# etzinis/sudo_rm_rf

Hardware: NVIDIA H100
Metric: mixtures_per_sec_forward_4s_8kHz_2src (higher is better)
Workload: dtype f32

## Files before the change

### sudo_rm_rf_b200/csrc/pointwise_mma.cu

```cuda
#include <cstdio>
#include <cstdlib>
#include <cstring>
#include <mutex>
#include <vector>
#include <cuda.h>
#include <cuda_bf16.h>
#include "common.cuh"

namespace sdr {

constexpr int kTileM = 128;
constexpr int kTileN = 128;
constexpr int kBlockK = 64;
constexpr int kStages = 3;
constexpr int kRawStages = 2;
constexpr int kBoxL = 32;
constexpr int kBoxBytes = 64 * kBoxL * 4;
constexpr int kRawStageBytes = kTileM / kBoxL * kBoxBytes;
constexpr int kBHalf = kTileN * 128;
constexpr int kBStageBytes = 2 * kBHalf;
constexpr int kSlotBytes = 2 * kBoxBytes;
constexpr int kSlots = 4;
constexpr int kConsWarps = 8, kTmaWarp = 8, kRawWarp = 9, kGatherWarps = 2;
template <bool WINDOW> constexpr int kMmaThreads = 32 * (kRawWarp + (WINDOW ? kGatherWarps : 1));

struct MmaArgs {
    const float* x;
    NormIn nin;
    const float* bias;
    int gate_channels;
    float* y;
    double* stats_out;
    int M, K, L;
    int l_tiles, n_tiles;
    int num_tiles;
    int epilogue;
    int win_k;
    int win_hop, win_pad, win_a;
    long long win_T;
};

__device__ __forceinline__ uint32_t smem_u32(const void* p) {
    return static_cast<uint32_t>(__cvta_generic_to_shared(p));
}
__device__ __forceinline__ void mbar_init(uint64_t* bar, uint32_t count) {
    asm volatile("mbarrier.init.shared::cta.b64 [%0], %1;" ::"r"(smem_u32(bar)), "r"(count) : "memory");
}
// ... 18 lines not shown
    asm volatile("fence.mbarrier_init.release.cluster;" ::: "memory");
}
__device__ __forceinline__ void fence_proxy_async_smem() {
    asm volatile("fence.proxy.async.shared::cta;" ::: "memory");
}
__device__ __forceinline__ void tma_load_2d(void* smem_dst, const CUtensorMap* tm, uint64_t* bar, int c0, int c1) {
    asm volatile("cp.async.bulk.tensor.2d.shared::cluster.global.tile.mbarrier::complete_tx::bytes [%0], [%1, {%3, %4}], [%2];"
                 ::"r"(smem_u32(smem_dst)), "l"(tm), "r"(smem_u32(bar)), "r"(c0), "r"(c1) : "memory");
}
__device__ __forceinline__ void tma_load_3d(void* smem_dst, const CUtensorMap* tm, uint64_t* bar, int c0, int c1, int c2) {
    asm volatile("cp.async.bulk.tensor.3d.shared::cluster.global.tile.mbarrier::complete_tx::bytes [%0], [%1, {%3, %4, %5}], [%2];"
                 ::"r"(smem_u32(smem_dst)), "l"(tm), "r"(smem_u32(bar)), "r"(c0), "r"(c1), "r"(c2) : "memory");
}
__device__ __forceinline__ void tma_store_3d(const CUtensorMap* tm, const void* smem_src, int c0, int c1, int c2) {
    asm volatile("cp.async.bulk.tensor.3d.global.shared::cta.bulk_group [%0, {%2, %3, %4}], [%1];"
                 ::"l"(tm), "r"(smem_u32(smem_src)), "r"(c0), "r"(c1), "r"(c2) : "memory");
}
__device__ __forceinline__ void bulk_commit() { asm volatile("cp.async.bulk.commit_group;" ::: "memory"); }
__device__ __forceinline__ void bulk_wait_read_all() { asm volatile("cp.async.bulk.wait_group.read 0;" ::: "memory"); }
__device__ __forceinline__ void bulk_wait_all() { asm volatile("cp.async.bulk.wait_group 0;" ::: "memory"); }
__device__ __forceinline__ void named_bar_sync(uint32_t id, uint32_t threads) {
    asm volatile("bar.sync %0, %1;" ::"r"(id), "r"(threads) : "memory");
}

__device__ __forceinline__ uint64_t gmma_desc_sw128(uint32_t saddr, uint32_t lbo, uint32_t sbo) {
    uint64_t d = 0;
    d |= (uint64_t)((saddr >> 4) & 0x3FFF);
    d |= (uint64_t)((lbo >> 4) & 0x3FFF) << 16;
    d |= (uint64_t)((sbo >> 4) & 0x3FFF) << 32;
    d |= (uint64_t)1 << 62;
    return d;
}
constexpr uint32_t kBLbo = 16, kBSbo = 1024;

__device__ __forceinline__ void wgmma_fence() { asm volatile("wgmma.fence.sync.aligned;" ::: "memory"); }
__device__ __forceinline__ void wgmma_commit() { asm volatile("wgmma.commit_group.sync.aligned;" ::: "memory"); }
template <int N>
__device__ __forceinline__ void wgmma_wait() { asm volatile("wgmma.wait_group.sync.aligned %0;" ::"n"(N) : "memory"); }
__device__ __forceinline__ void wgmma_bf16_m64n128_rs(float (&d)[64], const uint32_t (&a)[4], uint64_t bdesc,
                                                      uint32_t accumulate) {
    asm volatile(
        "{\n\t.reg .pred p;\n\t"
        "setp.ne.b32 p, %69, 0;\n\t"
        "wgmma.mma_async.sync.aligned.m64n128k16.f32.bf16.bf16 "
        "{%0, %1, %2, %3, %4, %5, %6, %7, %8, %9, %10, %11, %12, %13, %14, %15, %16, %17, %18, %19, %20, %21, %22, "
        "%23, %24, %25, %26, %27, %28, %29, %30, %31, %32, %33, %34, %35, %36, %37, %38, %39, %40, %41, %42, %43, %44, "
// ... 27 lines not shown
#pragma unroll
    for (int e = 0; e < 8; ++e) {
        const int k = kc * 8 + e;
        const float v = (m < M && k < Kreal) ? W[(size_t)m * Kreal + k] : 0.f;
        hi[e] = __float2bfloat16_rn(v);
        lo[e] = __float2bfloat16_rn(v - __bfloat162float(hi[e]));
    }
    *reinterpret_cast<uint4*>(img + off) = *reinterpret_cast<const uint4*>(hi);
    *reinterpret_cast<uint4*>(img + kBHalf + off) = *reinterpret_cast<const uint4*>(lo);
}

struct TileCoord { int sample, l0, n0; };
__device__ __forceinline__ TileCoord decode_tile(const MmaArgs& a, int tile) {
    TileCoord t;
    const int pos = tile / a.n_tiles;
    t.n0 = (tile - pos * a.n_tiles) * kTileN;
    t.sample = pos / a.l_tiles;
    t.l0 = (pos - t.sample * a.l_tiles) * kTileM;
    return t;
}

constexpr int kGroupSteps = 2;
constexpr int kGroups = kBlockK / 16 / kGroupSteps;
static_assert(kGroups == 2, "group g of every k-block uses fragment buffer g");
struct AFrag { uint32_t hi[kGroupSteps][4], lo[kGroupSteps][4]; };

template <bool WINDOW, int ACT, int MODE, bool STATS>
__global__ void __launch_bounds__(kMmaThreads<WINDOW>, 1)
pw_mma_kernel(const MmaArgs a, const __grid_constant__ CUtensorMap wmap,
              const __grid_constant__ CUtensorMap xmap,
              const __grid_constant__ CUtensorMap emap,
              const __grid_constant__ CUtensorMap ymap) {
    static_assert(!(WINDOW && ACT != 0), "the encoder's window operand has no activation");
    extern __shared__ uint8_t smem_raw[];
    uint8_t* smem = smem_raw + ((1024u - (smem_u32(smem_raw) & 1023u)) & 1023u);
    uint8_t* r_base = smem;
    uint8_t* b_base = r_base + kRawStages * kRawStageBytes;
    uint8_t* slots = b_base + kStages * kBStageBytes;
    float2* s_ab = reinterpret_cast<float2*>(slots + kSlots * kSlotBytes);
    float* s_sl = reinterpret_cast<float*>(s_ab + kRawStages * kBlockK);
    uint64_t* bars = reinterpret_cast<uint64_t*>(s_sl + kRawStages * kBlockK);
    uint64_t* full_bar = bars;
    uint64_t* empty_bar = full_bar + kStages;
    uint64_t* rfull_bar = empty_bar + kStages;
    uint64_t* rempty_bar = rfull_bar + kRawStages;
    uint64_t* slot_bar = rempty_bar + kRawStages;

    const int tid = threadIdx.x;
    const int warp = tid >> 5, lane = tid & 31;
    const int KB = a.K / kBlockK;
    const int tile0 = (int)blockIdx.x;
    const int tstep = (int)gridDim.x;

    if (warp == kTmaWarp && lane == 0) {
        for (int s = 0; s < kStages; ++s) { mbar_init(&full_bar[s], 1); mbar_init(&empty_bar[s], kConsWarps); }
        for (int s = 0; s < kRawStages; ++s) {
            mbar_init(&rfull_bar[s], WINDOW ? kGatherWarps : 2);
            mbar_init(&rempty_bar[s], kConsWarps);
        }
        for (int s = 0; s < kSlots; ++s) mbar_init(&slot_bar[s], 1);
        fence_barrier_init();
    }
    __syncthreads();

    if (warp >= kRawWarp) {
        int rs = 0;
        uint32_t rphase = 0;
        if constexpr (WINDOW) {
            constexpr int kGatherCh = kBlockK / kGatherWarps;
            const int c0 = (warp - kRawWarp) * kGatherCh;
#pragma unroll 1
            for (int tile = tile0; tile < a.num_tiles; tile += tstep) {
                const TileCoord tc = decode_tile(a, tile);
#pragma unroll 1
                for (int kb = 0; kb < KB; ++kb) {
                    uint8_t* rp = r_base + (size_t)rs * kRawStageBytes + (lane & 3) * 4;
#pragma unroll
                    for (int i0 = 0; i0 < kGatherCh; i0 += 16) {
                        float v[16][kTileM / kBoxL];
#pragma unroll
                        for (int i = 0; i < 16; ++i) {
                            const int k = kb * kBlockK + c0 + i0 + i;
                            const int ch = k / a.win_k, j = k - ch * a.win_k;
                            const float* src = a.x + ((size_t)tc.sample * a.win_a + ch) * a.win_T;
#pragma unroll
                            for (int b = 0; b < kTileM / kBoxL; ++b) {
                                const int l = tc.l0 + b * kBoxL + lane;
                                const long long t = (long long)a.win_hop * l + j - a.win_pad;
                                v[i][b] = (l < a.L && ch < a.win_a && t >= 0 && t < a.win_T) ? __ldg(src + t) : 0.f;
                            }
                        }
                        if (i0 == 0) mbar_wait(&rempty_bar[rs], rphase ^ 1);
#pragma unroll
                        for (int i = 0; i < 16; ++i) {
                            const int c = c0 + i0 + i;
#pragma unroll
                            for (int b = 0; b < kTileM / kBoxL; ++b)
                                *reinterpret_cast<float*>(rp + b * kBoxBytes + c * 128 + (((lane >> 2) ^ (c & 7)) << 4)) = v[i][b];
                        }
                    }
                    __syncwarp();
                    if (lane == 0) mbar_arrive(&rfull_bar[rs]);
                    if (++rs == kRawStages) { rs = 0; rphase ^= 1; }
                }
            }
        } else {
            const bool has_norm = a.nin.stats != nullptr;
            const double inv_count = 1.0 / a.nin.count;
#pragma unroll 1
            for (int tile = tile0; tile < a.num_tiles; tile += tstep) {
                const TileCoord tc = decode_tile(a, tile);
                float mean = 0.f, rstd = 1.f;
                if (has_norm) {
                    const double mu = a.nin.stats[2 * (size_t)tc.sample] * inv_count;
                    double var = a.nin.stats[2 * (size_t)tc.sample + 1] * inv_count - mu * mu;
                    var = var < 0.0 ? 0.0 : var;
                    mean = (float)mu;
                    rstd = rsqrtf((float)var + kGlnEps);
                }
#pragma unroll 1
                for (int kb = 0; kb < KB; ++kb) {
                    const int k = kb * kBlockK + 2 * lane;
                    float g[2] = {1.f, 1.f}, be[2] = {0.f, 0.f}, sl[2] = {1.f, 1.f};
                    if (has_norm) {
                        g[0] = __ldg(a.nin.gamma + k); g[1] = __ldg(a.nin.gamma + k + 1);
                        be[0] = __ldg(a.nin.beta + k); be[1] = __ldg(a.nin.beta + k + 1);
                    }
                    if constexpr (ACT == 2) { sl[0] = __ldg(a.nin.prelu + k); sl[1] = __ldg(a.nin.prelu + k + 1); }
                    mbar_wait(&rempty_bar[rs], rphase ^ 1);
                    if (lane == 0) {
                        mbar_arrive_expect_tx(&rfull_bar[rs], kRawStageBytes);
                        for (int b = 0; b < kTileM / kBoxL; ++b)
                            tma_load_3d(r_base + (size_t)rs * kRawStageBytes + b * kBoxBytes, &xmap, &rfull_bar[rs],
                                        tc.l0 + b * kBoxL, kb * kBlockK, tc.sample);
                    }
                    float aa[2] = {1.f, 1.f}, bb[2] = {0.f, 0.f};
                    if (has_norm) {
#pragma unroll
                        for (int e = 0; e < 2; ++e) { aa[e] = g[e] * rstd; bb[e] = be[e] - mean * aa[e]; }
                    }
                    *reinterpret_cast<float4*>(s_ab + rs * kBlockK + 2 * lane) = make_float4(aa[0], bb[0], aa[1], bb[1]);
                    if constexpr (ACT == 2) *reinterpret_cast<float2*>(s_sl + rs * kBlockK + 2 * lane) = make_float2(sl[0], sl[1]);
                    __syncwarp();
                    if (lane == 0) mbar_arrive(&rfull_bar[rs]);
                    if (++rs == kRawStages) { rs = 0; rphase ^= 1; }
                }
            }
        }
    } else if (warp == kTmaWarp) {
        if (lane == 0) {
            int stage = 0;
            uint32_t phase = 0;
            for (int tile = tile0; tile < a.num_tiles; tile += tstep) {
                const int nt = tile % a.n_tiles;
                for (int kb = 0; kb < KB; ++kb) {
                    mbar_wait(&empty_bar[stage], phase ^ 1);
                    mbar_arrive_expect_tx(&full_bar[stage], kBStageBytes);
                    tma_load_2d(b_base + (size_t)stage * kBStageBytes, &wmap, &full_bar[stage], 0, (nt * KB + kb) * 2 * kTileN);
                    if (++stage == kStages) { stage = 0; phase ^= 1; }
                }
            }
        }
        __syncwarp();
    } else {
        const int wg = warp >> 2;
        const int wr = warp & 3;
        const int q = lane & 3;
        const bool issuer = (tid & 127) == 0;
        const bool relu_out = WINDOW && a.epilogue == 2;
        const float slope = ACT == 1 ? __ldg(a.nin.prelu) : 1.f;
        const bool slope_le1 = slope <= 1.f;
        uint32_t boff[4];
#pragma unroll
        for (int v = 0; v < 4; ++v) {
            const uint32_t c = 2 * q + (v & 1), pp = 16 * (wr & 1) + (lane >> 2) + 8 * (v >> 1);
            boff[v] = c * 128 + (((pp >> 2) ^ c) << 4) + (pp & 3) * 4;
        }
        const uint32_t raw_box = (uint32_t)(2 * wg + (wr >> 1)) * kBoxBytes;
        uint8_t* const my_slots = slots + (size_t)(2 * wg) * kSlotBytes;
        auto fill_slot = [&](int tile, int h) {
            uint64_t* bar = &slot_bar[2 * wg + h];
            if constexpr (MODE == 0) {
                mbar_arrive(bar);
            } else {
                const TileCoord t = decode_tile(a, tile);
                const int c0 = t.l0 + 64 * wg;
                const int c1 = (MODE == 1 ? t.n0 : t.n0 % a.gate_channels) + 64 * h;
                uint8_t* const dst = my_slots + (size_t)h * kSlotBytes;
                mbar_arrive_expect_tx(bar, kSlotBytes);
                tma_load_3d(dst, &emap, bar, c0, c1, t.sample);
                tma_load_3d(dst + kBoxBytes, &emap, bar, c0 + kBoxL, c1, t.sample);
            }
        };
        if (issuer) { fill_slot(tile0, 0); fill_slot(tile0, 1); }

        int rs = 0, stage = 0, prev_stage = 0;
        uint32_t rphase = 0, phase = 0, slot_phase = 0;
        auto transform = [&](AFrag& f, int g) {
            if (g == 0) mbar_wait(&rfull_bar[rs], rphase);
            const uint8_t* rp = r_base + (size_t)rs * kRawStageBytes + raw_box;
            const float2* tab = s_ab + rs * kBlockK + 2 * q;
            const float* tsl = s_sl + rs * kBlockK + 2 * q;
#pragma unroll
            for (int s = 0; s < kGroupSteps; ++s) {
#pragma unroll
                for (int h = 0; h < 2; ++h) {
                    const int c = 16 * (g * kGroupSteps + s) + 8 * h;
                    float4 ab = make_float4(1.f, 0.f, 1.f, 0.f);
                    float2 sl = make_float2(1.f, 1.f);
                    if constexpr (!WINDOW) ab = *reinterpret_cast<const float4*>(tab + c);
                    if constexpr (ACT == 2) sl = *reinterpret_cast<const float2*>(tsl + c);
#pragma unroll
                    for (int ph = 0; ph < 2; ++ph) {
                        float y[2];
#pragma unroll
                        for (int e = 0; e < 2; ++e) {
                            const float x = *reinterpret_cast<const float*>(rp + boff[e + 2 * ph] + c * 128);
                            y[e] = WINDOW ? x : fmaf(x, e ? ab.z : ab.x, e ? ab.w : ab.y);
                            if constexpr (ACT == 1) {
                                const float t = y[e] * slope;
                                y[e] = slope_le1 ? fmaxf(y[e], t) : fminf(y[e], t);
                            } else if constexpr (ACT == 2) {
                                y[e] = y[e] >= 0.f ? y[e] : y[e] * (e ? sl.y : sl.x);
                            }
                        }
                        const uint32_t h0 = __float_as_uint(y[0]) & 0xffff0000u, h1 = __float_as_uint(y[1]) & 0xffff0000u;
                        const __nv_bfloat162 lo = __floats2bfloat162_rn(y[0] - __uint_as_float(h0), y[1] - __uint_as_float(h1));
                        f.hi[s][2 * h + ph] = __byte_perm(h0, h1, 0x7632);
                        f.lo[s][2 * h + ph] = *reinterpret_cast<const uint32_t*>(&lo);
                    }
                }
            }
            if (g == kGroups - 1) {
                __syncwarp();
                if (lane == 0) mbar_arrive(&rempty_bar[rs]);
                if (++rs == kRawStages) { rs = 0; rphase ^= 1; }
            }
        };
        float acc[64];
        auto mma_group = [&](int kb, int g, const AFrag& cur, AFrag& nxt) {
            if (g == 0) mbar_wait(&full_bar[stage], phase);
            const uint32_t sb_hi = smem_u32(b_base + (size_t)stage * kBStageBytes);
            const uint32_t sb_lo = sb_hi + kBHalf;
            wgmma_fence();
#pragma unroll
            for (int s = 0; s < kGroupSteps; ++s) {
                const int ks = g * kGroupSteps + s;
                const uint64_t dbh = gmma_desc_sw128(sb_hi + ks * 32, kBLbo, kBSbo);
                const uint64_t dbl = gmma_desc_sw128(sb_lo + ks * 32, kBLbo, kBSbo);
                wgmma_bf16_m64n128_rs(acc, cur.hi[s], dbh, (kb | ks) != 0 ? 1u : 0u);
                wgmma_bf16_m64n128_rs(acc, cur.lo[s], dbh, 1u);
                wgmma_bf16_m64n128_rs(acc, cur.hi[s], dbl, 1u);
            }
            wgmma_commit();
            wgmma_wait<1>();
            if (g == 0 && kb > 0) {
                __syncwarp();
                if (lane == 0) mbar_arrive(&empty_bar[prev_stage]);
            }
            if (g == kGroups - 1) {
                prev_stage = stage;
                if (++stage == kStages) { stage = 0; phase ^= 1; }
                if (kb + 1 < KB) transform(nxt, 0);
            } else {
                transform(nxt, g + 1);
            }
        };
        AFrag fa, fb;
#pragma unroll 1
        for (int tile = tile0; tile < a.num_tiles; tile += tstep) {
            const TileCoord tc = decode_tile(a, tile);
#pragma unroll
            for (int i = 0; i < 64; ++i) acc[i] = 0.f;
            transform(fa, 0);
#pragma unroll 1
            for (int kb = 0; kb < KB; ++kb) {
                mma_group(kb, 0, fa, fb);
                mma_group(kb, 1, fb, fa);
            }
            wgmma_wait<0>();
            __syncwarp();
            if (lane == 0) mbar_arrive(&empty_bar[prev_stage]);
            const int prem = a.L - (tc.l0 + wg * 64 + 32 * (wr >> 1) + 16 * (wr & 1) + (lane >> 2));
            StatAcc st;
            float rs_ = 0.f, rq = 0.f;
#pragma unroll
            for (int h = 0; h < 2; ++h) {
                uint8_t* const slot = my_slots + (size_t)h * kSlotBytes;
                uint8_t* const box = slot + (wr >> 1) * kBoxBytes;
                const int m0 = tc.n0 + 64 * h + 2 * q;
                const int mrem = a.M - m0;
                mbar_wait(&slot_bar[2 * wg + h], slot_phase);
#pragma unroll
                for (int j = 0; j < 8; ++j) {
                    float bv[2];
#pragma unroll
                    for (int b = 0; b < 2; ++b) bv[b] = (a.bias && 8 * j + b < mrem) ? __ldg(a.bias + m0 + 8 * j + b) : 0.f;
#pragma unroll
                    for (int v = 0; v < 4; ++v) {
                        const int u = 4 * j + v, i = 32 * h + u;
                        float* e = reinterpret_cast<float*>(box + boff[v] + 1024 * j);
                        float o = acc[i] + bv[v & 1];
                        if (MODE == 1) o += *e;
                        if (MODE == 2) o = fmaxf(o, 0.f) * *e;
                        if constexpr (WINDOW) { if (relu_out) o = fmaxf(o, 0.f); }
                        *e = o;
                        if (STATS && 8 * j + (v & 1) < mrem && 8 * (v >> 1) < prem) { rs_ += o; rq = fmaf(o, o, rq); }
                        if (STATS && (i & 15) == 15) { st.add_run(rs_, rq); rs_ = rq = 0.f; }
                    }
                }
                if constexpr (WINDOW) {
                    named_bar_sync(1 + wg, 128);
#pragma unroll 4
                    for (int r = wr; r < 64; r += 4) {
                        const int m = tc.n0 + 64 * h + r;
#pragma unroll
                        for (int half = 0; half < 2; ++half) {
                            const int p = tc.l0 + wg * 64 + half * kBoxL + lane;
                            const float v = *reinterpret_cast<const float*>(
                                slot + half * kBoxBytes + r * 128 + (((lane >> 2) ^ (r & 7)) << 4) + (lane & 3) * 4);
                            if (m < a.M && p < a.L) a.y[((size_t)tc.sample * a.M + m) * a.L + p] = v;
                        }
                    }
                    named_bar_sync(1 + wg, 128);
                } else {
                    fence_proxy_async_smem();
                    named_bar_sync(1 + wg, 128);
                    if (issuer) {
                        const int c0 = tc.l0 + wg * 64, c1 = tc.n0 + 64 * h;
                        tma_store_3d(&ymap, slot, c0, c1, tc.sample);
                        tma_store_3d(&ymap, slot + kBoxBytes, c0 + kBoxL, c1, tc.sample);
                        bulk_commit();
                        bulk_wait_read_all();
                    }
                }
                if (issuer && tile + tstep < a.num_tiles) fill_slot(tile + tstep, h);
            }
            slot_phase ^= 1;
            if (STATS) {
                const double ds = warp_sum_f64(st.s), dq = warp_sum_f64(st.q);
                if (lane == 0) {
                    atomicAdd(a.stats_out + 2 * (size_t)tc.sample, ds);
                    atomicAdd(a.stats_out + 2 * (size_t)tc.sample + 1, dq);
                }
            }
        }
        if (!WINDOW && issuer) bulk_wait_all();
    }
}

static inline int mma_pad_m(int M) { return (M + kTileN - 1) / kTileN * kTileN; }

bool pointwise_mma_eligible(int M, int K) {
    return M >= 32 && K >= kBlockK && (K % kBlockK) == 0;
}

size_t pointwise_mma_packed_bytes(int M, int K) {
    if (!pointwise_mma_eligible(M, K)) return 0;
    return (size_t)mma_pad_m(M) * K * 4;
}

// ... 39 lines not shown
                           CU_TENSOR_MAP_L2_PROMOTION_L2_256B, CU_TENSOR_MAP_FLOAT_OOB_FILL_NONE);
    return r == CUDA_SUCCESS ? SDR_OK : SDR_ERR_UNSUPPORTED;
}

static int make_act_map(CUtensorMap* tm, const float* x, int samples, int C, int L) {
    memset(tm, 0, sizeof(*tm));
    EncodeTiledFn enc = encode_tiled_fn();
    if (!enc) return SDR_ERR_CUDA;
    const cuuint64_t dims[3] = {(cuuint64_t)L, (cuuint64_t)C, (cuuint64_t)samples};
    const cuuint64_t strides[2] = {(cuuint64_t)L * 4, (cuuint64_t)L * C * 4};
    const cuuint32_t box[3] = {(cuuint32_t)kBoxL, 64, 1};
    const cuuint32_t estr[3] = {1, 1, 1};
    const CUresult r = enc(tm, CU_TENSOR_MAP_DATA_TYPE_FLOAT32, 3, const_cast<float*>(x), dims, strides, box, estr,
                           CU_TENSOR_MAP_INTERLEAVE_NONE, CU_TENSOR_MAP_SWIZZLE_128B,
                           CU_TENSOR_MAP_L2_PROMOTION_L2_256B, CU_TENSOR_MAP_FLOAT_OOB_FILL_NONE);
    return r == CUDA_SUCCESS ? SDR_OK : SDR_ERR_UNSUPPORTED;
}
static_assert(kBlockK == 64 && kTileN == 2 * 64, "activation boxes are 64 channels: one k-block, half a channel tile");

struct MmaLaunchInfo { const void* fn; int dev; int sms; };
static std::mutex g_launch_mutex;
static std::vector<MmaLaunchInfo> g_launch_info;

template <bool WINDOW, typename Kern>
static int launch_persistent(Kern kern, const MmaArgs& a, const CUtensorMap& wmap, const CUtensorMap& xmap,
                             const CUtensorMap& emap, const CUtensorMap& ymap, cudaStream_t st) {
    int dev = 0;
    if (cudaGetDevice(&dev) != cudaSuccess) return SDR_ERR_CUDA;
    int sms = 0;
    {
        std::lock_guard<std::mutex> lock(g_launch_mutex);
        for (const MmaLaunchInfo& e : g_launch_info)
            if (e.fn == reinterpret_cast<const void*>(kern) && e.dev == dev) { sms = e.sms; break; }
        if (sms == 0) {
            if (cudaFuncSetAttribute(kern, cudaFuncAttributeMaxDynamicSharedMemorySize, (int)kMmaSmemBytes) != cudaSuccess) {
                cudaGetLastError();
                return SDR_ERR_CUDA;
            }
            if (cudaDeviceGetAttribute(&sms, cudaDevAttrMultiProcessorCount, dev) != cudaSuccess || sms <= 0) return SDR_ERR_CUDA;
            g_launch_info.push_back(MmaLaunchInfo{reinterpret_cast<const void*>(kern), dev, sms});
        }
    }
    const int grid = a.num_tiles < sms ? a.num_tiles : sms;
    kern<<<grid, kMmaThreads<WINDOW>, kMmaSmemBytes, st>>>(a, wmap, xmap, emap, ymap);
    if (cudaGetLastError() != cudaSuccess) return SDR_ERR_CUDA;
    return SDR_OK;
}

int launch_pointwise_mma(const float* x, const NormIn& nin, const void* wpk, const float* bias,
                         const float* residual, const float* gate, int gate_channels,
                         float* y, double* stats_out, int samples, int M, int K, int L,
                         int epilogue, cudaStream_t st) {
    auto misaligned = [](const float* p) { return (reinterpret_cast<uintptr_t>(p) % 16) != 0; };
    if (!pointwise_mma_eligible(M, K) || (L % 4) != 0 || misaligned(x) || misaligned(y) ||
        (epilogue != 1 && misaligned(residual)) || (epilogue == 1 && misaligned(gate)))
        return SDR_ERR_UNSUPPORTED;
    if (samples <= 0 || L <= 0 || !x || !wpk || !y) return SDR_ERR_BAD_ARGUMENT;
    if (epilogue == 1 && (!gate || gate_channels <= 0)) return SDR_ERR_BAD_ARGUMENT;
    if (epilogue == 1 && (gate_channels % kTileN) != 0) return SDR_ERR_UNSUPPORTED;
    if (reinterpret_cast<uintptr_t>(wpk) % 16) return SDR_ERR_BAD_ARGUMENT;
    MmaArgs a;
    a.x = x; a.nin = nin; a.bias = bias;
    a.gate_channels = gate_channels; a.y = y; a.stats_out = stats_out;
    a.M = M; a.K = K; a.L = L; a.epilogue = epilogue;
    a.win_k = 0; a.win_hop = 0; a.win_pad = 0; a.win_a = 0; a.win_T = 0;
    a.n_tiles = mma_pad_m(M) / kTileN;
    a.l_tiles = (L + kTileM - 1) / kTileM;
    const long long tiles = (long long)samples * a.l_tiles * a.n_tiles;
    if (tiles > 0x7fffffffLL) return SDR_ERR_UNSUPPORTED;
    a.num_tiles = (int)tiles;
    const int act = nin.prelu ? (nin.prelu_pc ? 2 : 1) : 0;
    const int mode = epilogue == 1 ? 2 : (residual ? 1 : 0);
    const bool stats = stats_out != nullptr;
    CUtensorMap wmap, xmap, emap, ymap;
    if (int rc = make_weight_map(&wmap, wpk, pointwise_mma_packed_bytes(M, K))) return rc;
    if (int rc = make_act_map(&xmap, x, samples, K, L)) return rc;
    if (int rc = make_act_map(&ymap, y, samples, M, L)) return rc;
    memset(&emap, 0, sizeof(emap));
    if (mode == 1)
        if (int rc = make_act_map(&emap, residual, samples, M, L)) return rc;
    if (mode == 2)
        if (int rc = make_act_map(&emap, gate, samples, gate_channels, L)) return rc;
#define SDR_MMA_CASE(A, MD, ST)                                                                                   \
    if (act == A && mode == MD && stats == ST)                                                                    \
        return launch_persistent<false>(pw_mma_kernel<false, A, MD, ST>, a, wmap, xmap, emap, ymap, st);
    SDR_MMA_CASE(0, 0, false) SDR_MMA_CASE(0, 0, true)
    SDR_MMA_CASE(1, 0, false) SDR_MMA_CASE(1, 0, true)
    SDR_MMA_CASE(0, 1, false) SDR_MMA_CASE(0, 1, true)
    SDR_MMA_CASE(1, 1, false) SDR_MMA_CASE(1, 1, true)
    SDR_MMA_CASE(0, 2, false) SDR_MMA_CASE(0, 2, true)
    SDR_MMA_CASE(1, 2, false) SDR_MMA_CASE(1, 2, true)
    SDR_MMA_CASE(2, 0, false) SDR_MMA_CASE(2, 0, true)
#undef SDR_MMA_CASE
    return SDR_ERR_UNSUPPORTED;
}

static inline int enc_kpad(int A, int Kk) { return (A * Kk + kBlockK - 1) / kBlockK * kBlockK; }

size_t encoder_mma_packed_bytes(int N, int A, int Kk) {
    if (N < 32 || A < 1 || Kk < 3) return 0;
    return (size_t)mma_pad_m(N) * enc_kpad(A, Kk) * 4;
}

int pack_encoder_mma(const float* W, int N, int A, int Kk, void* packed, cudaStream_t st) {
    if (!encoder_mma_packed_bytes(N, A, Kk)) return SDR_ERR_UNSUPPORTED;
    const int Mpad = mma_pad_m(N), K = enc_kpad(A, Kk);
    const long long chunks = (long long)Mpad * K / 8;
    pack_weight_mma_kernel<<<(unsigned)((chunks + 255) / 256), 256, 0, st>>>(
        W, static_cast<uint8_t*>(packed), N, Mpad, A * Kk, K);
    return cudaGetLastError() == cudaSuccess ? SDR_OK : SDR_ERR_CUDA;
}

int launch_encoder_mma(const float* wav, const void* wpk, const float* bias, int relu, float* enc, double* stats,
                       int B, int A, long long T, int N, int Kk, int L, int pad, cudaStream_t st) {
    if (!encoder_mma_packed_bytes(N, A, Kk)) return SDR_ERR_UNSUPPORTED;
    if (B <= 0 || T <= 0 || L <= 0 || !wav || !wpk || !enc) return SDR_ERR_BAD_ARGUMENT;
    MmaArgs a;
    a.x = wav; a.nin = NormIn{nullptr, nullptr, nullptr, nullptr, 1.0};
    a.bias = bias;
    a.gate_channels = 0; a.y = enc; a.stats_out = stats;
    a.M = N; a.K = enc_kpad(A, Kk); a.L = L; a.epilogue = relu ? 2 : 0;
    a.win_k = Kk; a.win_hop = Kk / 2; a.win_pad = pad; a.win_a = A; a.win_T = T;
    a.n_tiles = mma_pad_m(N) / kTileN;
    a.l_tiles = (L + kTileM - 1) / kTileM;
    const long long tiles = (long long)B * a.l_tiles * a.n_tiles;
    if (tiles > 0x7fffffffLL) return SDR_ERR_UNSUPPORTED;
    a.num_tiles = (int)tiles;
    CUtensorMap wmap, none;
    if (int rc = make_weight_map(&wmap, wpk, encoder_mma_packed_bytes(N, A, Kk))) return rc;
    memset(&none, 0, sizeof(none));
    if (stats) return launch_persistent<true>(pw_mma_kernel<true, 0, 0, true>, a, wmap, none, none, none, st);
    return launch_persistent<true>(pw_mma_kernel<true, 0, 0, false>, a, wmap, none, none, none, st);
}

}
```

Before: 2003.

## Add ping-pong consumer warpgroup schedule with register redistribution for pointwise GEMM

Adds a ping-pong variant of the persistent pointwise WGMMA kernel. Each consumer warpgroup owns whole tiles and alternates between two accumulator sets, so one tile's epilogue can overlap another tile's MMA. Producer warps give up registers via setmaxnreg so the consumers can hold two accumulator sets. The variant runs when K spans at most eight blocks and there are at least two tiles per SM; it adds register pressure and more complex slot and barrier handling.

New measurement: 2050, median of 6. 1.02x the previous value.

```diff
diff --git a/sudo_rm_rf_b200/csrc/pointwise_mma.cu b/sudo_rm_rf_b200/csrc/pointwise_mma.cu
--- a/sudo_rm_rf_b200/csrc/pointwise_mma.cu
+++ b/sudo_rm_rf_b200/csrc/pointwise_mma.cu
@@ -2,6 +2,7 @@
 #include <cstdlib>
 #include <cstring>
 #include <mutex>
+#include <utility>
 #include <vector>
 #include <cuda.h>
 #include <cuda_bf16.h>
@@ -21,8 +22,10 @@
 constexpr int kBStageBytes = 2 * kBHalf;
 constexpr int kSlotBytes = 2 * kBoxBytes;
 constexpr int kSlots = 4;
-constexpr int kConsWarps = 8, kTmaWarp = 8, kRawWarp = 9, kGatherWarps = 2;
-template <bool WINDOW> constexpr int kMmaThreads = 32 * (kRawWarp + (WINDOW ? kGatherWarps : 1));
+constexpr int kWgWarps = 4, kTmaWarp = 8, kRawWarp = 9, kGatherWarps = 2;
+template <bool WINDOW, bool PP> constexpr int kMmaThreads = PP ? 384 : 32 * (kRawWarp + (WINDOW ? kGatherWarps : 1));
+constexpr int kConsRegs = 232, kProdRegs = 40;
+static_assert(2 * kConsRegs + kProdRegs == 3 * 168, "setmaxnreg redistributes exactly the launch allocation");
 
 struct MmaArgs {
     const float* x;
@@ -87,6 +90,26 @@
 __device__ __forceinline__ void named_bar_sync(uint32_t id, uint32_t threads) {
     asm volatile("bar.sync %0, %1;" ::"r"(id), "r"(threads) : "memory");
 }
+__device__ __forceinline__ void named_bar_arrive(uint32_t id, uint32_t threads) {
+    asm volatile("bar.arrive %0, %1;" ::"r"(id), "r"(threads) : "memory");
+}
+template <int N> __device__ __forceinline__ void setmaxnreg_inc() { asm volatile("setmaxnreg.inc.sync.aligned.u32 %0;" ::"n"(N)); }
+__device__ __forceinline__ int thread_idx() {
+    int t;
+    asm volatile("mov.u32 %0, %%tid.x;" : "=r"(t));
+    return t;
+}
+__device__ __forceinline__ int cta_idx() {
+    int t;
+    asm volatile("mov.u32 %0, %%ctaid.x;" : "=r"(t));
+    return t;
+}
+__device__ __forceinline__ int grid_ctas() {
+    int t;
+    asm volatile("mov.u32 %0, %%nctaid.x;" : "=r"(t));
+    return t;
+}
+template <int N> __device__ __forceinline__ void setmaxnreg_dec() { asm volatile("setmaxnreg.dec.sync.aligned.u32 %0;" ::"n"(N)); }
 
 __device__ __forceinline__ uint64_t gmma_desc_sw128(uint32_t saddr, uint32_t lbo, uint32_t sbo) {
     uint64_t d = 0;
@@ -160,16 +183,18 @@
 
 constexpr int kGroupSteps = 2;
 constexpr int kGroups = kBlockK / 16 / kGroupSteps;
-static_assert(kGroups == 2, "group g of every k-block uses fragment buffer g");
-struct AFrag { uint32_t hi[kGroupSteps][4], lo[kGroupSteps][4]; };
-
-template <bool WINDOW, int ACT, int MODE, bool STATS>
-__global__ void __launch_bounds__(kMmaThreads<WINDOW>, 1)
+static_assert(kGroups % 2 == 0, "groups alternate between the two fragment buffers");
+template <int SETS> struct AFrag { uint32_t hi[SETS][kGroupSteps][4], lo[SETS][kGroupSteps][4]; };
+
+template <bool WINDOW, int ACT, int MODE, bool STATS, bool PP = false>
+__global__ void __launch_bounds__(kMmaThreads<WINDOW, PP>, 1)
 pw_mma_kernel(const MmaArgs a, const __grid_constant__ CUtensorMap wmap,
               const __grid_constant__ CUtensorMap xmap,
               const __grid_constant__ CUtensorMap emap,
               const __grid_constant__ CUtensorMap ymap) {
     static_assert(!(WINDOW && ACT != 0), "the encoder's window operand has no activation");
+    static_assert(!(WINDOW && PP), "the encoder runs split tiles");
+    constexpr int kStageConsumers = PP ? kWgWarps : 2 * kWgWarps;
     extern __shared__ uint8_t smem_raw[];
     uint8_t* smem = smem_raw + ((1024u - (smem_u32(smem_raw) & 1023u)) & 1023u);
     uint8_t* r_base = smem;
@@ -184,125 +209,135 @@
     uint64_t* rempty_bar = rfull_bar + kRawStages;
     uint64_t* slot_bar = rempty_bar + kRawStages;
 
-    const int tid = threadIdx.x;
-    const int warp = tid >> 5, lane = tid & 31;
+    const int warp = threadIdx.x >> 5;
     const int KB = a.K / kBlockK;
-    const int tile0 = (int)blockIdx.x;
-    const int tstep = (int)gridDim.x;
-
-    if (warp == kTmaWarp && lane == 0) {
-        for (int s = 0; s < kStages; ++s) { mbar_init(&full_bar[s], 1); mbar_init(&empty_bar[s], kConsWarps); }
+
+    if (threadIdx.x == kTmaWarp * 32) {
+        for (int s = 0; s < kStages; ++s) { mbar_init(&full_bar[s], 1); mbar_init(&empty_bar[s], kStageConsumers); }
         for (int s = 0; s < kRawStages; ++s) {
             mbar_init(&rfull_bar[s], WINDOW ? kGatherWarps : 2);
-            mbar_init(&rempty_bar[s], kConsWarps);
+            mbar_init(&rempty_bar[s], kStageConsumers);
         }
         for (int s = 0; s < kSlots; ++s) mbar_init(&slot_bar[s], 1);
         fence_barrier_init();
     }
     __syncthreads();
 
-    if (warp >= kRawWarp) {
-        int rs = 0;
-        uint32_t rphase = 0;
-        if constexpr (WINDOW) {
-            constexpr int kGatherCh = kBlockK / kGatherWarps;
-            const int c0 = (warp - kRawWarp) * kGatherCh;
+    if (warp >= kTmaWarp) {
+        if constexpr (PP) setmaxnreg_dec<kProdRegs>();
+        const int tile0 = cta_idx(), tstep = grid_ctas();
+        const int lane = thread_idx() & 31;
+        if (warp >= kRawWarp + (WINDOW ? kGatherWarps : 1)) {
+        } else if (warp >= kRawWarp) {
+            int rs = 0;
+            uint32_t rphase = 0;
+            if constexpr (WINDOW) {
+                constexpr int kGatherCh = kBlockK / kGatherWarps;
+                constexpr int kGatherBatch = 16;
+                const int c0 = (warp - kRawWarp) * kGatherCh;
 #pragma unroll 1
-            for (int tile = tile0; tile < a.num_tiles; tile += tstep) {
-                const TileCoord tc = decode_tile(a, tile);
+                for (int tile = tile0; tile < a.num_tiles; tile += tstep) {
+                    const TileCoord tc = decode_tile(a, tile);
 #pragma unroll 1
-                for (int kb = 0; kb < KB; ++kb) {
-                    uint8_t* rp = r_base + (size_t)rs * kRawStageBytes + (lane & 3) * 4;
-#pragma unroll
-                    for (int i0 = 0; i0 < kGatherCh; i0 += 16) {
-                        float v[16][kTileM / kBoxL];
-#pragma unroll
-                        for (int i = 0; i < 16; ++i) {
-                            const int k = kb * kBlockK + c0 + i0 + i;
-                            const int ch = k / a.win_k, j = k - ch * a.win_k;
-                            const float* src = a.x + ((size_t)tc.sample * a.win_a + ch) * a.win_T;
-#pragma unroll
-                            for (int b = 0; b < kTileM / kBoxL; ++b) {
-                                const int l = tc.l0 + b * kBoxL + lane;
-                                const long long t = (long long)a.win_hop * l + j - a.win_pad;
-                                v[i][b] = (l < a.L && ch < a.win_a && t >= 0 && t < a.win_T) ? __ldg(src + t) : 0.f;
+                    for (int kb = 0; kb < KB; ++kb) {
+                        uint8_t* rp = r_base + (size_t)rs * kRawStageBytes + (lane & 3) * 4;
+#pragma unroll
+                        for (int i0 = 0; i0 < kGatherCh; i0 += kGatherBatch) {
+                            float v[kGatherBatch][kTileM / kBoxL];
+#pragma unroll
+                            for (int i = 0; i < kGatherBatch; ++i) {
+                                const int k = kb * kBlockK + c0 + i0 + i;
+                                const int ch = k / a.win_k, j = k - ch * a.win_k;
+                                const float* src = a.x + ((size_t)tc.sample * a.win_a + ch) * a.win_T;
+#pragma unroll
+                                for (int b = 0; b < kTileM / kBoxL; ++b) {
+                                    const int l = tc.l0 + b * kBoxL + lane;
+                                    const long long t = (long long)a.win_hop * l + j - a.win_pad;
+                                    v[i][b] = (l < a.L && ch < a.win_a && t >= 0 && t < a.win_T) ? __ldg(src + t) : 0.f;
+                                }
+                            }
+                            if (i0 == 0) mbar_wait(&rempty_bar[rs], rphase ^ 1);
+#pragma unroll
+                            for (int i = 0; i < kGatherBatch; ++i) {
+                                const int c = c0 + i0 + i;
+#pragma unroll
+                                for (int b = 0; b < kTileM / kBoxL; ++b)
+                                    *reinterpret_cast<float*>(rp + b * kBoxBytes + c * 128 + (((lane >> 2) ^ (c & 7)) << 4)) = v[i][b];
                             }
                         }
-                        if (i0 == 0) mbar_wait(&rempty_bar[rs], rphase ^ 1);
-#pragma unroll
-                        for (int i = 0; i < 16; ++i) {
-                            const int c = c0 + i0 + i;
-#pragma unroll
+                        __syncwarp();
+                        if (lane == 0) mbar_arrive(&rfull_bar[rs]);
+                        if (++rs == kRawStages) { rs = 0; rphase ^= 1; }
+                    }
+                }
+            } else {
+                const bool has_norm = a.nin.stats != nullptr;
+                const double inv_count = 1.0 / a.nin.count;
+#pragma unroll 1
+                for (int tile = tile0; tile < a.num_tiles; tile += tstep) {
+                    const TileCoord tc = decode_tile(a, tile);
+                    float mean = 0.f, rstd = 1.f;
+                    if (has_norm) {
+                        const double mu = a.nin.stats[2 * (size_t)tc.sample] * inv_count;
+                        double var = a.nin.stats[2 * (size_t)tc.sample + 1] * inv_count - mu * mu;
+                        var = var < 0.0 ? 0.0 : var;
+                        mean = (float)mu;
+                        rstd = rsqrtf((float)var + kGlnEps);
+                    }
+#pragma unroll 1
+                    for (int kb = 0; kb < KB; ++kb) {
+                        const int k = kb * kBlockK + 2 * lane;
+                        float g[2] = {1.f, 1.f}, be[2] = {0.f, 0.f}, sl[2] = {1.f, 1.f};
+                        if (has_norm) {
+                            g[0] = __ldg(a.nin.gamma + k); g[1] = __ldg(a.nin.gamma + k + 1);
+                            be[0] = __ldg(a.nin.beta + k); be[1] = __ldg(a.nin.beta + k + 1);
+                        }
+                        if constexpr (ACT == 2) { sl[0] = __ldg(a.nin.prelu + k); sl[1] = __ldg(a.nin.prelu + k + 1); }
+                        mbar_wait(&rempty_bar[rs], rphase ^ 1);
+                        if (lane == 0) {
+                            mbar_arrive_expect_tx(&rfull_bar[rs], kRawStageBytes);
                             for (int b = 0; b < kTileM / kBoxL; ++b)
-                                *reinterpret_cast<float*>(rp + b * kBoxBytes + c * 128 + (((lane >> 2) ^ (c & 7)) << 4)) = v[i][b];
+                                tma_load_3d(r_base + (size_t)rs * kRawStageBytes + b * kBoxBytes, &xmap, &rfull_bar[rs],
+                                            tc.l0 + b * kBoxL, kb * kBlockK, tc.sample);
                         }
+                        float aa[2] = {1.f, 1.f}, bb[2] = {0.f, 0.f};
+                        if (has_norm) {
+#pragma unroll
+                            for (int e = 0; e < 2; ++e) { aa[e] = g[e] * rstd; bb[e] = be[e] - mean * aa[e]; }
+                        }
+                        *reinterpret_cast<float4*>(s_ab + rs * kBlockK + 2 * lane) = make_float4(aa[0], bb[0], aa[1], bb[1]);
+                        if constexpr (ACT == 2) *reinterpret_cast<float2*>(s_sl + rs * kBlockK + 2 * lane) = make_float2(sl[0], sl[1]);
+                        __syncwarp();
+                        if (lane == 0) mbar_arrive(&rfull_bar[rs]);
+                        if (++rs == kRawStages) { rs = 0; rphase ^= 1; }
                     }
-                    __syncwarp();
-                    if (lane == 0) mbar_arrive(&rfull_bar[rs]);
-                    if (++rs == kRawStages) { rs = 0; rphase ^= 1; }
                 }
             }
-        } else {
-            const bool has_norm = a.nin.stats != nullptr;
-            const double inv_count = 1.0 / a.nin.count;
-#pragma unroll 1
-            for (int tile = tile0; tile < a.num_tiles; tile += tstep) {
-                const TileCoord tc = decode_tile(a, tile);
-                float mean = 0.f, rstd = 1.f;
-                if (has_norm) {
-                    const double mu = a.nin.stats[2 * (size_t)tc.sample] * inv_count;
-                    double var = a.nin.stats[2 * (size_t)tc.sample + 1] * inv_count - mu * mu;
-                    var = var < 0.0 ? 0.0 : var;
-                    mean = (float)mu;
-                    rstd = rsqrtf((float)var + kGlnEps);
+        } else if (warp == kTmaWarp) {
+            if (lane == 0) {
+                int stage = 0;
+                uint32_t phase = 0;
+                for (int tile = tile0; tile < a.num_tiles; tile += tstep) {
+                    const int nt = tile % a.n_tiles;
+                    for (int kb = 0; kb < KB; ++kb) {
+                        mbar_wait(&empty_bar[stage], phase ^ 1);
+                        mbar_arrive_expect_tx(&full_bar[stage], kBStageBytes);
+                        tma_load_2d(b_base + (size_t)stage * kBStageBytes, &wmap, &full_bar[stage], 0, (nt * KB + kb) * 2 * kTileN);
+                        if (++stage == kStages) { stage = 0; phase ^= 1; }
+                    }
                 }
-#pragma unroll 1
-                for (int kb = 0; kb < KB; ++kb) {
-                    const int k = kb * kBlockK + 2 * lane;
-                    float g[2] = {1.f, 1.f}, be[2] = {0.f, 0.f}, sl[2] = {1.f, 1.f};
-                    if (has_norm) {
-                        g[0] = __ldg(a.nin.gamma + k); g[1] = __ldg(a.nin.gamma + k + 1);
-                        be[0] = __ldg(a.nin.beta + k); be[1] = __ldg(a.nin.beta + k + 1);
-                    }
-                    if constexpr (ACT == 2) { sl[0] = __ldg(a.nin.prelu + k); sl[1] = __ldg(a.nin.prelu + k + 1); }
-                    mbar_wait(&rempty_bar[rs], rphase ^ 1);
-                    if (lane == 0) {
-                        mbar_arrive_expect_tx(&rfull_bar[rs], kRawStageBytes);
-                        for (int b = 0; b < kTileM / kBoxL; ++b)
-                            tma_load_3d(r_base + (size_t)rs * kRawStageBytes + b * kBoxBytes, &xmap, &rfull_bar[rs],
-                                        tc.l0 + b * kBoxL, kb * kBlockK, tc.sample);
-                    }
-                    float aa[2] = {1.f, 1.f}, bb[2] = {0.f, 0.f};
-                    if (has_norm) {
-#pragma unroll
-                        for (int e = 0; e < 2; ++e) { aa[e] = g[e] * rstd; bb[e] = be[e] - mean * aa[e]; }
-                    }
-                    *reinterpret_cast<float4*>(s_ab + rs * kBlockK + 2 * lane) = make_float4(aa[0], bb[0], aa[1], bb[1]);
-                    if constexpr (ACT == 2) *reinterpret_cast<float2*>(s_sl + rs * kBlockK + 2 * lane) = make_float2(sl[0], sl[1]);
-                    __syncwarp();
-                    if (lane == 0) mbar_arrive(&rfull_bar[rs]);
-                    if (++rs == kRawStages) { rs = 0; rphase ^= 1; }
-                }
-            }
+            }
+            __syncwarp();
         }
-    } else if (warp == kTmaWarp) {
-        if (lane == 0) {
-            int stage = 0;
-            uint32_t phase = 0;
-            for (int tile = tile0; tile < a.num_tiles; tile += tstep) {
-                const int nt = tile % a.n_tiles;
-                for (int kb = 0; kb < KB; ++kb) {
-                    mbar_wait(&empty_bar[stage], phase ^ 1);
-                    mbar_arrive_expect_tx(&full_bar[stage], kBStageBytes);
-                    tma_load_2d(b_base + (size_t)stage * kBStageBytes, &wmap, &full_bar[stage], 0, (nt * KB + kb) * 2 * kTileN);
-                    if (++stage == kStages) { stage = 0; phase ^= 1; }
-                }
-            }
-        }
-        __syncwarp();
     } else {
+        if constexpr (PP) setmaxnreg_inc<kConsRegs>();
+        const int tile0 = cta_idx(), tstep = grid_ctas();
+        const int tid = thread_idx(), lane = tid & 31;
+        constexpr int kSets = PP ? 2 : 1;
         const int wg = warp >> 2;
         const int wr = warp & 3;
+        auto half_of = [&](int set) { return PP ? set : wg; };
+        const int tile_step = PP ? 2 * tstep : tstep;
         const int q = lane & 3;
         const bool issuer = (tid & 127) == 0;
         const bool relu_out = WINDOW && a.epilogue == 2;
@@ -314,15 +349,15 @@
             const uint32_t c = 2 * q + (v & 1), pp = 16 * (wr & 1) + (lane >> 2) + 8 * (v >> 1);
             boff[v] = c * 128 + (((pp >> 2) ^ c) << 4) + (pp & 3) * 4;
         }
-        const uint32_t raw_box = (uint32_t)(2 * wg + (wr >> 1)) * kBoxBytes;
+        const uint32_t raw_box = (uint32_t)(wr >> 1) * kBoxBytes;
         uint8_t* const my_slots = slots + (size_t)(2 * wg) * kSlotBytes;
-        auto fill_slot = [&](int tile, int h) {
+        auto fill_slot = [&](int tile, int hf, int h) {
             uint64_t* bar = &slot_bar[2 * wg + h];
             if constexpr (MODE == 0) {
                 mbar_arrive(bar);
             } else {
                 const TileCoord t = decode_tile(a, tile);
-                const int c0 = t.l0 + 64 * wg;
+                const int c0 = t.l0 + 64 * hf;
                 const int c1 = (MODE == 1 ? t.n0 : t.n0 % a.gate_channels) + 64 * h;
                 uint8_t* const dst = my_slots + (size_t)h * kSlotBytes;
                 mbar_arrive_expect_tx(bar, kSlotBytes);
@@ -330,11 +365,19 @@
                 tma_load_3d(dst + kBoxBytes, &emap, bar, c0 + kBoxL, c1, t.sample);
             }
         };
-        if (issuer) { fill_slot(tile0, 0); fill_slot(tile0, 1); }
+        const int first = PP ? tile0 + wg * tstep : tile0;
+        if (issuer && first < a.num_tiles) { fill_slot(first, half_of(0), 0); fill_slot(first, half_of(0), 1); }
 
         int rs = 0, stage = 0, prev_stage = 0;
         uint32_t rphase = 0, phase = 0, slot_phase = 0;
-        auto transform = [&](AFrag& f, int g) {
+        auto skip_tile = [&]() {
+            rphase ^= ((rs + KB) / kRawStages) & 1;
+            rs = (rs + KB) % kRawStages;
+            phase ^= ((stage + KB) / kStages) & 1;
+            stage = (stage + KB) % kStages;
+        };
+        if (PP && wg == 1) skip_tile();
+        auto transform = [&](AFrag<kSets>& f, int g) {
             if (g == 0) mbar_wait(&rfull_bar[rs], rphase);
             const uint8_t* rp = r_base + (size_t)rs * kRawStageBytes + raw_box;
             const float2* tab = s_ab + rs * kBlockK + 2 * q;
@@ -349,23 +392,26 @@
                     if constexpr (!WINDOW) ab = *reinterpret_cast<const float4*>(tab + c);
                     if constexpr (ACT == 2) sl = *reinterpret_cast<const float2*>(tsl + c);
 #pragma unroll
-                    for (int ph = 0; ph < 2; ++ph) {
-                        float y[2];
-#pragma unroll
-                        for (int e = 0; e < 2; ++e) {
-                            const float x = *reinterpret_cast<const float*>(rp + boff[e + 2 * ph] + c * 128);
-                            y[e] = WINDOW ? x : fmaf(x, e ? ab.z : ab.x, e ? ab.w : ab.y);
-                            if constexpr (ACT == 1) {
-                                const float t = y[e] * slope;
-                                y[e] = slope_le1 ? fmaxf(y[e], t) : fminf(y[e], t);
-                            } else if constexpr (ACT == 2) {
-                                y[e] = y[e] >= 0.f ? y[e] : y[e] * (e ? sl.y : sl.x);
+                    for (int hp = 0; hp < kSets; ++hp) {
+#pragma unroll
+                        for (int ph = 0; ph < 2; ++ph) {
+                            float y[2];
+#pragma unroll
+                            for (int e = 0; e < 2; ++e) {
+                                const float x = *reinterpret_cast<const float*>(rp + 2 * half_of(hp) * kBoxBytes + boff[e + 2 * ph] + c * 128);
+                                y[e] = WINDOW ? x : fmaf(x, e ? ab.z : ab.x, e ? ab.w : ab.y);
+                                if constexpr (ACT == 1) {
+                                    const float t = y[e] * slope;
+                                    y[e] = slope_le1 ? fmaxf(y[e], t) : fminf(y[e], t);
+                                } else if constexpr (ACT == 2) {
+                                    y[e] = y[e] >= 0.f ? y[e] : y[e] * (e ? sl.y : sl.x);
+                                }
                             }
+                            const uint32_t h0 = __float_as_uint(y[0]) & 0xffff0000u, h1 = __float_as_uint(y[1]) & 0xffff0000u;
+                            const __nv_bfloat162 lo = __floats2bfloat162_rn(y[0] - __uint_as_float(h0), y[1] - __uint_as_float(h1));
+                            f.hi[hp][s][2 * h + ph] = __byte_perm(h0, h1, 0x7632);
+                            f.lo[hp][s][2 * h + ph] = *reinterpret_cast<const uint32_t*>(&lo);
                         }
-                        const uint32_t h0 = __float_as_uint(y[0]) & 0xffff0000u, h1 = __float_as_uint(y[1]) & 0xffff0000u;
-                        const __nv_bfloat162 lo = __floats2bfloat162_rn(y[0] - __uint_as_float(h0), y[1] - __uint_as_float(h1));
-                        f.hi[s][2 * h + ph] = __byte_perm(h0, h1, 0x7632);
-                        f.lo[s][2 * h + ph] = *reinterpret_cast<const uint32_t*>(&lo);
                     }
                 }
             }
@@ -375,8 +421,8 @@
                 if (++rs == kRawStages) { rs = 0; rphase ^= 1; }
             }
         };
-        float acc[64];
-        auto mma_group = [&](int kb, int g, const AFrag& cur, AFrag& nxt) {
+        float acc[kSets][64];
+        auto mma_group = [&](int kb, int g, const AFrag<kSets>& cur, AFrag<kSets>& nxt) {
             if (g == 0) mbar_wait(&full_bar[stage], phase);
             const uint32_t sb_hi = smem_u32(b_base + (size_t)stage * kBStageBytes);
             const uint32_t sb_lo = sb_hi + kBHalf;
@@ -386,9 +432,12 @@
                 const int ks = g * kGroupSteps + s;
                 const uint64_t dbh = gmma_desc_sw128(sb_hi + ks * 32, kBLbo, kBSbo);
                 const uint64_t dbl = gmma_desc_sw128(sb_lo + ks * 32, kBLbo, kBSbo);
-                wgmma_bf16_m64n128_rs(acc, cur.hi[s], dbh, (kb | ks) != 0 ? 1u : 0u);
-                wgmma_bf16_m64n128_rs(acc, cur.lo[s], dbh, 1u);
-                wgmma_bf16_m64n128_rs(acc, cur.hi[s], dbl, 1u);
+#pragma unroll
+                for (int hp = 0; hp < kSets; ++hp) {
+                    wgmma_bf16_m64n128_rs(acc[hp], cur.hi[hp][s], dbh, (kb | ks) != 0 ? 1u : 0u);
+                    wgmma_bf16_m64n128_rs(acc[hp], cur.lo[hp][s], dbh, 1u);
+                    wgmma_bf16_m64n128_rs(acc[hp], cur.hi[hp][s], dbl, 1u);
+                }
             }
             wgmma_commit();
             wgmma_wait<1>();
@@ -404,77 +453,93 @@
                 transform(nxt, g + 1);
             }
         };
-        AFrag fa, fb;
+        AFrag<kSets> fa, fb;
 #pragma unroll 1
-        for (int tile = tile0; tile < a.num_tiles; tile += tstep) {
+        for (int tile = first; tile < a.num_tiles; tile += tile_step) {
             const TileCoord tc = decode_tile(a, tile);
 #pragma unroll
-            for (int i = 0; i < 64; ++i) acc[i] = 0.f;
+            for (int i = 0; i < 64; ++i) {
+#pragma unroll
+                for (int hp = 0; hp < kSets; ++hp) acc[hp][i] = 0.f;
+            }
+            if (PP && tile != tile0) named_bar_sync(3 + wg, 256);
             transform(fa, 0);
 #pragma unroll 1
             for (int kb = 0; kb < KB; ++kb) {
-                mma_group(kb, 0, fa, fb);
-                mma_group(kb, 1, fb, fa);
+#pragma unroll
+                for (int g = 0; g < kGroups; g += 2) {
+                    mma_group(kb, g, fa, fb);
+                    if (PP && g == 0 && kb == KB - 1 && tile + tstep < a.num_tiles)
+                        named_bar_arrive(3 + (wg ^ 1), 256);
+                    mma_group(kb, g + 1, fb, fa);
+                }
             }
             wgmma_wait<0>();
             __syncwarp();
             if (lane == 0) mbar_arrive(&empty_bar[prev_stage]);
-            const int prem = a.L - (tc.l0 + wg * 64 + 32 * (wr >> 1) + 16 * (wr & 1) + (lane >> 2));
+            if constexpr (PP) skip_tile();
             StatAcc st;
             float rs_ = 0.f, rq = 0.f;
 #pragma unroll
-            for (int h = 0; h < 2; ++h) {
-                uint8_t* const slot = my_slots + (size_t)h * kSlotBytes;
-                uint8_t* const box = slot + (wr >> 1) * kBoxBytes;
-                const int m0 = tc.n0 + 64 * h + 2 * q;
-                const int mrem = a.M - m0;
-                mbar_wait(&slot_bar[2 * wg + h], slot_phase);
-#pragma unroll
-                for (int j = 0; j < 8; ++j) {
-                    float bv[2];
-#pragma unroll
-                    for (int b = 0; b < 2; ++b) bv[b] = (a.bias && 8 * j + b < mrem) ? __ldg(a.bias + m0 + 8 * j + b) : 0.f;
-#pragma unroll
-                    for (int v = 0; v < 4; ++v) {
-                        const int u = 4 * j + v, i = 32 * h + u;
-                        float* e = reinterpret_cast<float*>(box + boff[v] + 1024 * j);
-                        float o = acc[i] + bv[v & 1];
-                        if (MODE == 1) o += *e;
-                        if (MODE == 2) o = fmaxf(o, 0.f) * *e;
-                        if constexpr (WINDOW) { if (relu_out) o = fmaxf(o, 0.f); }
-                        *e = o;
-                        if (STATS && 8 * j + (v & 1) < mrem && 8 * (v >> 1) < prem) { rs_ += o; rq = fmaf(o, o, rq); }
-                        if (STATS && (i & 15) == 15) { st.add_run(rs_, rq); rs_ = rq = 0.f; }
+            for (int ph = 0; ph < kSets; ++ph) {
+                const int prem = a.L - (tc.l0 + 64 * half_of(ph) + 32 * (wr >> 1) + 16 * (wr & 1) + (lane >> 2));
+#pragma unroll
+                for (int h = 0; h < 2; ++h) {
+                    uint8_t* const slot = my_slots + (size_t)h * kSlotBytes;
+                    uint8_t* const box = slot + (wr >> 1) * kBoxBytes;
+                    const int m0 = tc.n0 + 64 * h + 2 * q;
+                    const int mrem = a.M - m0;
+                    mbar_wait(&slot_bar[2 * wg + h], slot_phase);
+#pragma unroll
+                    for (int j = 0; j < 8; ++j) {
+                        float bv[2];
+#pragma unroll
+                        for (int b = 0; b < 2; ++b) bv[b] = (a.bias && 8 * j + b < mrem) ? __ldg(a.bias + m0 + 8 * j + b) : 0.f;
+#pragma unroll
+                        for (int v = 0; v < 4; ++v) {
+                            const int u = 4 * j + v, i = 32 * h + u;
+                            float* e = reinterpret_cast<float*>(box + boff[v] + 1024 * j);
+                            float o = acc[ph][i] + bv[v & 1];
+                            if (MODE == 1) o += *e;
+                            if (MODE == 2) o = fmaxf(o, 0.f) * *e;
+                            if constexpr (WINDOW) { if (relu_out) o = fmaxf(o, 0.f); }
+                            *e = o;
+                            if (STATS && 8 * j + (v & 1) < mrem && 8 * (v >> 1) < prem) { rs_ += o; rq = fmaf(o, o, rq); }
+                            if (STATS && (i & 15) == 15) { st.add_run(rs_, rq); rs_ = rq = 0.f; }
+                        }
+                    }
+                    if constexpr (WINDOW) {
+                        named_bar_sync(1 + wg, 128);
+#pragma unroll 4
+                        for (int r = wr; r < 64; r += 4) {
+                            const int m = tc.n0 + 64 * h + r;
+#pragma unroll
+                            for (int half = 0; half < 2; ++half) {
+                                const int p = tc.l0 + 64 * half_of(ph) + half * kBoxL + lane;
+                                const float v = *reinterpret_cast<const float*>(
+                                    slot + half * kBoxBytes + r * 128 + (((lane >> 2) ^ (r & 7)) << 4) + (lane & 3) * 4);
+                                if (m < a.M && p < a.L) a.y[((size_t)tc.sample * a.M + m) * a.L + p] = v;
+                            }
+                        }
+                        named_bar_sync(1 + wg, 128);
+                    } else {
+                        fence_proxy_async_smem();
+                        named_bar_sync(1 + wg, 128);
+                        if (issuer) {
+                            const int c0 = tc.l0 + 64 * half_of(ph), c1 = tc.n0 + 64 * h;
+                            tma_store_3d(&ymap, slot, c0, c1, tc.sample);
+                            tma_store_3d(&ymap, slot + kBoxBytes, c0 + kBoxL, c1, tc.sample);
+                            bulk_commit();
+                            bulk_wait_read_all();
+                        }
+                    }
+                    if (issuer) {
+                        if (PP && ph == 0) fill_slot(tile, 1, h);
+                        else if (tile + tile_step < a.num_tiles) fill_slot(tile + tile_step, half_of(0), h);
                     }
                 }
-                if constexpr (WINDOW) {
-                    named_bar_sync(1 + wg, 128);
-#pragma unroll 4
-                    for (int r = wr; r < 64; r += 4) {
-                        const int m = tc.n0 + 64 * h + r;
-#pragma unroll
-                        for (int half = 0; half < 2; ++half) {
-                            const int p = tc.l0 + wg * 64 + half * kBoxL + lane;
-                            const float v = *reinterpret_cast<const float*>(
-                                slot + half * kBoxBytes + r * 128 + (((lane >> 2) ^ (r & 7)) << 4) + (lane & 3) * 4);
-                            if (m < a.M && p < a.L) a.y[((size_t)tc.sample * a.M + m) * a.L + p] = v;
-                        }
-                    }
-                    named_bar_sync(1 + wg, 128);
-                } else {
-                    fence_proxy_async_smem();
-                    named_bar_sync(1 + wg, 128);
-                    if (issuer) {
-                        const int c0 = tc.l0 + wg * 64, c1 = tc.n0 + 64 * h;
-                        tma_store_3d(&ymap, slot, c0, c1, tc.sample);
-                        tma_store_3d(&ymap, slot + kBoxBytes, c0 + kBoxL, c1, tc.sample);
-                        bulk_commit();
-                        bulk_wait_read_all();
-                    }
-                }
-                if (issuer && tile + tstep < a.num_tiles) fill_slot(tile + tstep, h);
-            }
-            slot_phase ^= 1;
+                slot_phase ^= 1;
+            }
             if (STATS) {
                 const double ds = warp_sum_f64(st.s), dq = warp_sum_f64(st.q);
                 if (lane == 0) {
@@ -560,7 +625,19 @@
 static std::mutex g_launch_mutex;
 static std::vector<MmaLaunchInfo> g_launch_info;
 
-template <bool WINDOW, typename Kern>
+static int device_sms(int* sms) {
+    static std::vector<std::pair<int, int>> cache;
+    int dev = 0;
+    if (cudaGetDevice(&dev) != cudaSuccess) return SDR_ERR_CUDA;
+    std::lock_guard<std::mutex> lock(g_launch_mutex);
+    for (const auto& e : cache)
+        if (e.first == dev) { *sms = e.second; return SDR_OK; }
+    if (cudaDeviceGetAttribute(sms, cudaDevAttrMultiProcessorCount, dev) != cudaSuccess || *sms <= 0) return SDR_ERR_CUDA;
+    cache.emplace_back(dev, *sms);
+    return SDR_OK;
+}
+
+template <bool WINDOW, bool PP, typename Kern>
 static int launch_persistent(Kern kern, const MmaArgs& a, const CUtensorMap& wmap, const CUtensorMap& xmap,
                              const CUtensorMap& emap, const CUtensorMap& ymap, cudaStream_t st) {
     int dev = 0;
@@ -580,7 +657,7 @@
         }
     }
     const int grid = a.num_tiles < sms ? a.num_tiles : sms;
-    kern<<<grid, kMmaThreads<WINDOW>, kMmaSmemBytes, st>>>(a, wmap, xmap, emap, ymap);
+    kern<<<grid, kMmaThreads<WINDOW, PP>, kMmaSmemBytes, st>>>(a, wmap, xmap, emap, ymap);
     if (cudaGetLastError() != cudaSuccess) return SDR_ERR_CUDA;
     return SDR_OK;
 }
@@ -619,9 +696,13 @@
         if (int rc = make_act_map(&emap, residual, samples, M, L)) return rc;
     if (mode == 2)
         if (int rc = make_act_map(&emap, gate, samples, gate_channels, L)) return rc;
+    int sms = 0;
+    if (int rc = device_sms(&sms)) return rc;
+    const bool pp = K / kBlockK <= 8 && a.num_tiles >= 2 * sms;
 #define SDR_MMA_CASE(A, MD, ST)                                                                                   \
     if (act == A && mode == MD && stats == ST)                                                                    \
-        return launch_persistent<false>(pw_mma_kernel<false, A, MD, ST>, a, wmap, xmap, emap, ymap, st);
+        return pp ? launch_persistent<false, true>(pw_mma_kernel<false, A, MD, ST, true>, a, wmap, xmap, emap, ymap, st) \
+                  : launch_persistent<false, false>(pw_mma_kernel<false, A, MD, ST, false>, a, wmap, xmap, emap, ymap, st);
     SDR_MMA_CASE(0, 0, false) SDR_MMA_CASE(0, 0, true)
     SDR_MMA_CASE(1, 0, false) SDR_MMA_CASE(1, 0, true)
     SDR_MMA_CASE(0, 1, false) SDR_MMA_CASE(0, 1, true)
@@ -667,8 +748,8 @@
     CUtensorMap wmap, none;
     if (int rc = make_weight_map(&wmap, wpk, encoder_mma_packed_bytes(N, A, Kk))) return rc;
     memset(&none, 0, sizeof(none));
-    if (stats) return launch_persistent<true>(pw_mma_kernel<true, 0, 0, true>, a, wmap, none, none, none, st);
-    return launch_persistent<true>(pw_mma_kernel<true, 0, 0, false>, a, wmap, none, none, none, st);
-}
-
-}
+    if (stats) return launch_persistent<true, false>(pw_mma_kernel<true, 0, 0, true>, a, wmap, none, none, none, st);
+    return launch_persistent<true, false>(pw_mma_kernel<true, 0, 0, false>, a, wmap, none, none, none, st);
+}
+
+}
```
